# BartvLaatum/GreenLight-Gym2

Hardware: NVIDIA B200
Metric: GreenLight env-steps/sec (fp64 parity) (higher is better)
Workload: dtype f64

## Files before the change

### greenlight-gym2_b200/csrc/glg_kernels.cuh

```cuda
#pragma once
#include <cuda_runtime.h>
#include <stdint.h>

#include "glg_controller.h"
#include "glg_model.h"
#include "glg_philox.h"
#include "glg_rk4.h"

#define GLG_NOBS_FIXED 23
#define GLG_MAXOBSMOD 8
#define GLG_OBS_STATE 1
#define GLG_OBS_CLIMATE 2
#define GLG_OBS_CROP 3
#define GLG_OBS_CONTROL 4
#define GLG_OBS_WEATHER 5
#define GLG_OBS_TIME 6
#define GLG_OBS_FORECAST 7
#define GLG_NOBS_STATE 27
#define GLG_NINFO 11
#define GLG_NSTATS 16

struct GlgUniform {
    double P[GLG_NP];
    double K[K_COUNT];
// ... 160 lines not shown
                if (off + i < 3) o3[off + i] = v;
            }
        } else if (id == GLG_OBS_STATE) {
#pragma unroll 1
            for (int b = 0; b < (GLG_NOBS_STATE + 1) / 2; ++b) {
                const GlgPhilox4 r = glg_philox4x32_10(96u + (uint32_t)b, ctr, (uint32_t)env_id, (uint32_t)(env_id >> 32),
                                                       (uint32_t)A.seed, (uint32_t)(A.seed >> 32));
                const double v0 = glg_u01(r.v[0], r.v[1]), v1 = glg_u01(r.v[2], r.v[3]);
                orow[off + 2 * b] = (float)v0;
                if (hrow) hrow[hoff + 2 * b] = (float)v0;
                if (off + 2 * b < 3) o3[off + 2 * b] = v0;
                if (2 * b + 1 < GLG_NOBS_STATE) {
                    orow[off + 2 * b + 1] = (float)v1;
                    if (hrow) hrow[hoff + 2 * b + 1] = (float)v1;
                    if (off + 2 * b + 1 < 3) o3[off + 2 * b + 1] = v1;
                }
            }
        } else if (id == GLG_OBS_FORECAST) {
#pragma unroll 1
            for (int i = 0; off + i < 3 && i < 5 * A.Np; ++i) o3[off + i] = wnext[(i / 5) * GLG_ND + (i % 5)];
        }
    }
}

__device__ __forceinline__ double glg_warp_sum(double v) {
#pragma unroll
    for (int o = 16; o > 0; o >>= 1) v += __shfl_down_sync(0xffffffffu, v, o);
    return v;
}


__device__ __forceinline__ int glg_stage_weather(const GlgStepArgs &A, double *s_wtile, uint64_t *s_bar, int *s_misc,
                                                 bool active, int kw, int tbl, int &bk, int &bt) {
    if (threadIdx.x == 0) {
        s_misc[0] = kw;
        s_misc[1] = tbl;
        glg_mbar_init(s_bar, 1);
    }
    __syncthreads();
    bk = s_misc[0];
    bt = s_misc[1];
    const int uniform = __syncthreads_and(!active || (kw == bk && tbl == bt));
    if (uniform) {
        const uint32_t tile_bytes = (uint32_t)((A.Np + 1) * GLG_ND * sizeof(double));
        if (threadIdx.x == 0) {
            glg_mbar_expect_tx(s_bar, tile_bytes);
            glg_bulk_g2s(s_wtile, A.weather + ((size_t)bt * A.rows + (size_t)bk) * GLG_ND, tile_bytes, s_bar);
        }
        glg_mbar_wait(s_bar, 0);
    }
    return uniform;
}

template <bool NOISY, class HC, class CC>
__device__ __forceinline__ void glg_env_prologue(const GlgUniform &U, const GlgStepArgs &A, int e, const double *wrow,
                                                 unsigned int ctr, HC &Hc, CC &Cc, double *x, double *u, double *d) {
    const int B = A.B;
#pragma unroll
    for (int i = 0; i < 7; ++i) d[i] = wrow[i];
    if (A.raw_control == 2) {
        double xc[GLG_NX], dc[GLG_ND];
#pragma unroll
        for (int i = 0; i < GLG_NX; ++i) xc[i] = (i == 0 || i == 2 || i == 15) ? A.x[(size_t)i * B + e] : 0.0;
#pragma unroll
        for (int i = 0; i < GLG_ND; ++i) dc[i] = wrow[i];
        glg_rule_control(A.ctrl, xc, dc, A.time[(size_t)B + e], A.time[e], u);
    } else if (A.raw_control) {
#pragma unroll
        for (int i = 0; i < GLG_NU; ++i) u[i] = A.controls[(size_t)e * GLG_NU + i];
    } else {
#pragma unroll
        for (int i = 0; i < GLG_NU; ++i) {
            const float prod = __fmul_rn(A.actions[(size_t)e * GLG_NU + i], A.delta_u_max_f32);
            u[i] = glg_clamp(A.u[(size_t)i * B + e] + (double)prod, A.u_min[i], A.u_max[i]);
        }
    }
#pragma unroll
    for (int i = 0; i < GLG_NU; ++i) A.u[(size_t)i * B + e] = u[i];
#pragma unroll
    for (int i = 0; i < GLG_NX; ++i) x[i] = A.x[(size_t)i * B + e];
    if (NOISY) {
        double pl[GLG_NP];
        double n34[34];
        if (A.noise) {
#pragma unroll 1
            for (int i = 0; i < 34; ++i) n34[i] = A.noise[(size_t)e * 34 + i];
        } else {
            glg_noise34(A.seed, (unsigned long long)(A.env_id_offset + e), ctr, A.uncertainty_scale, n34);
        }
#pragma unroll 1
        for (int i = 0; i < GLG_NP; ++i) pl[i] = U.P[i];
#pragma unroll 1
        for (int i = 0; i < 34; ++i) {
            const double pv = U.P[128 + i];
            pl[128 + i] = (double)__double2float_rn(pv + n34[i] * pv);
        }
        pl[144] = (double)__fdiv_rn(__double2float_rn(pl[141]), __double2float_rn(pl[142]));
        double Cl[C_COUNT];
        glg_make_c(pl, Cl);
#pragma unroll
        for (int i = 0; i < C_COUNT; ++i) Cc[i] = Cl[i];
        glg_hoist(pl, u, d, Hc);
    } else {
        glg_hoist(GlgConstView{U.P}, u, d, Hc);
    }
}

struct GlgEnvOut {
    int done, k_obs, tbl_obs, k_term, tbl_term;
    double fin_ret, fin_len, fin_info[GLG_NINFO];
};

__device__ __forceinline__ void glg_env_epilogue(const GlgUniform &U, const GlgStepArgs &A, int e, int k, int kw, int tbl,
                                                 const double *wrow, double *x, double fruit_prev, int bad,
                                                 unsigned int ctr, GlgEnvOut &o) {
    const int B = A.B;
    const size_t table_stride = (size_t)A.rows * GLG_ND;
    int done = 0;
    if (bad) {
#pragma unroll
        for (int i = 0; i < GLG_NX; ++i) x[i] = A.x[(size_t)i * B + e];
        done = 1;
    }
    double doy = A.time[e], hod = A.time[(size_t)B + e];
    doy += fmod(A.dt / 86400.0, 365.0);
    hod = fmod(hod + A.dt / 3600.0, 24.0);
    double u[GLG_NU], d[GLG_ND];
#pragma unroll
    for (int i = 0; i < GLG_NU; ++i) u[i] = A.u[(size_t)i * B + e];
#pragma unroll
    for (int i = 0; i < 5; ++i) d[i] = wrow[i];
    double hd[GLG_NOBS_FIXED];
    double o3[3] = {0.0, 0.0, 0.0};
    glg_obs_head(x, u, d, k, doy, hod, hd);
    float *orow = A.obs + (size_t)e * A.obs_dim;
    const unsigned long long env_gid = (unsigned long long)(A.env_id_offset + e);
    float *step_row = orow;
    float *hrow = A.obs_head + (size_t)e * (A.obs_dim - (A.fc_off >= 0 ? 5 * A.Np : 0));
    if (k >= A.N) done = 1;
    if (done && A.auto_reset) step_row = A.term_obs + (size_t)e * A.obs_dim;
    glg_write_obs_row(A, hd, wrow + GLG_ND, env_gid, ctr, step_row, step_row == orow ? hrow : nullptr, o3);
    double reward, info[GLG_NINFO];
    {
        const double dt = A.dt;
        const double heat_costs = u[0] * U.P[108] / U.P[46] * dt / 3600 * 1e-3 * A.heating_price;
        const double elec_costs = u[4] * U.P[172] * dt / 3600 * 1e-3 * A.elec_price;
        const double co2_costs = u[1] * U.P[109] / U.P[46] * dt * 1e-6 * A.co2_price;
        const double variable_costs = 0 + heat_costs + co2_costs + elec_costs;
        const double gains = (x[25] - fruit_prev) * 1e-6 / A.dmfm * A.fruit_price;
        const double profit = gains - variable_costs;
        const double max_profit = U.P[154] * dt * 1e-6 / A.dmfm * A.fruit_price;
        const double max_heating = U.P[108] / U.P[46] * dt / 3600 * 1e-3 * A.heating_price;
        const double max_elec = U.P[172] * dt / 3600 * 1e-3 * A.elec_price;
        const double max_co2 = U.P[109] / U.P[46] * dt * 1e-6 * A.co2_price;
        const double min_profit = -(0 + max_heating + max_elec + max_co2);
        const double max_viol[3] = {2500, 15, 15};
        double viol[3], pen = 0.0;
#pragma unroll
// ... 40 lines not shown
        doy = A.start_day[tbl];
        hod = 0.0;
        glg_obs_head(x, u, d, 0, doy, hod, hd);
        double o3r[3];
        glg_write_obs_row(A, hd, w0 + GLG_ND, env_gid, ctr + 0x80000000u, orow, hrow, o3r);
        o.k_obs = 0;
        o.tbl_obs = tbl;
    }
#pragma unroll
    for (int i = 0; i < GLG_NX; ++i) A.x[(size_t)i * B + e] = x[i];
    A.timestep[e] = k;
    A.table[e] = tbl;
    A.time[e] = doy;
    A.time[(size_t)B + e] = hod;
    A.step_ctr[e] = ctr + 1u;
    A.ep_return[e] = done ? 0.0 : ep_ret;
    A.ep_len[e] = done ? 0 : ep_len;
#pragma unroll
    for (int j = 0; j < GLG_NINFO; ++j) A.ep_info[(size_t)j * B + e] = done ? 0.0 : info[j];
    o.done = done;
    o.fin_ret = done ? ep_ret : 0.0;
    o.fin_len = done ? (double)ep_len : 0.0;
#pragma unroll
    for (int j = 0; j < GLG_NINFO; ++j) o.fin_info[j] = done ? info[j] : 0.0;
}

__device__ __forceinline__ void glg_stats_reduce(const GlgStepArgs &A, bool active, int bad, const GlgEnvOut &o) {
    const unsigned any_done = __ballot_sync(0xffffffffu, active && o.done);
    if (!any_done) return;
    const double cnt = glg_warp_sum((active && o.done) ? 1.0 : 0.0);
    const double ret = glg_warp_sum(o.fin_ret);
    const double len = glg_warp_sum(o.fin_len);
    const double nbad = glg_warp_sum((active && bad) ? 1.0 : 0.0);
    double isum[GLG_NINFO];
#pragma unroll
    for (int j = 0; j < GLG_NINFO; ++j) isum[j] = glg_warp_sum(o.fin_info[j]);
    if ((threadIdx.x & 31) == 0) {
        atomicAdd(A.stats + 0, cnt);
        atomicAdd(A.stats + 1, ret);
        atomicAdd(A.stats + 2, len);
#pragma unroll
        for (int j = 0; j < GLG_NINFO; ++j) atomicAdd(A.stats + 3 + j, isum[j]);
        atomicAdd(A.stats + 14, nbad);
    }
}

__device__ __forceinline__ void glg_write_forecast(const GlgStepArgs &A, int NR, const int *s_tbl, const int *s_k,
                                                   const int *s_tbl_t, const int *s_k_t, const double *s_wtile,
                                                   int uniform, int bk, int bt) {
    if (A.fc_off < 0) return;
    const size_t table_stride = (size_t)A.rows * GLG_ND;
    const int nf = 5 * A.Np;
    const int row0 = blockIdx.x * NR;
#pragma unroll 1
    for (int r = 0; r < NR; ++r) {
        const int kk = s_k[r];
        if (kk < 0) continue;
        const int tb = s_tbl[r];
        const double *src = (uniform && tb == bt && kk == bk) ? s_wtile : (A.weather + (size_t)tb * table_stride + (size_t)kk * GLG_ND);
        float *orow = A.obs + (size_t)(row0 + r) * A.obs_dim + A.fc_off;
        for (int j = threadIdx.x; j < nf; j += blockDim.x) {
            const int i = j / 5, c = j - 5 * i;
            orow[j] = (float)src[(size_t)(1 + i) * GLG_ND + c];
        }
        const int kt = s_k_t[r];
        if (kt >= 0) {
            const double *srct = A.weather + (size_t)s_tbl_t[r] * table_stride + (size_t)kt * GLG_ND;
            float *trow = A.term_obs + (size_t)(row0 + r) * A.obs_dim + A.fc_off;
            for (int j = threadIdx.x; j < nf; j += blockDim.x) {
                const int i = j / 5, c = j - 5 * i;
                trow[j] = (float)srct[(size_t)(1 + i) * GLG_ND + c];
            }
        }
    }
}

template <int NT, bool NOISY>
struct GlgStepSmem {
    static constexpr int kColRows = 2 * GLG_NX + H_COUNT + (NOISY ? C_COUNT : 0);
    __host__ __device__ static size_t bytes(int Np) {
        return sizeof(double) * ((size_t)kColRows * NT + (size_t)(Np + 1) * GLG_ND) + 16  + sizeof(int) * (4 * NT + 4);
    }
};

template <bool GENERAL, bool NOISY, int NT>
__global__ void __launch_bounds__(NT) glg_step_kernel(const __grid_constant__ GlgUniform U, const __grid_constant__ GlgStepArgs A) {
    glg_exp_tbl_fill();
    extern __shared__ __align__(16) unsigned char smem_raw[];
    double *s_wtile = reinterpret_cast<double *>(smem_raw);
    double *s_cols = s_wtile + (size_t)(A.Np + 1) * GLG_ND;
    uint64_t *s_bar = reinterpret_cast<uint64_t *>(s_cols + (size_t)GlgStepSmem<NT, NOISY>::kColRows * NT);
    int *s_tbl = reinterpret_cast<int *>(s_bar + 2);
    int *s_k = s_tbl + NT;
    int *s_tbl_t = s_k + NT;
    int *s_k_t = s_tbl_t + NT;
    int *s_misc = s_k_t + NT;

    const int tid = threadIdx.x;
    const int e = blockIdx.x * NT + tid;
    const bool active = e < A.B;
    int k = 0, tbl = 0;
    if (active) {
        k = A.timestep[e];
        tbl = A.table[e];
    }
    const int kw = min(k, A.rows - A.Np - 1);
    int bk, bt;
    const int uniform = glg_stage_weather(A, s_wtile, s_bar, s_misc, active, kw, tbl, bk, bt);

    GlgEnvOut o;
    o.done = 0; o.k_obs = -1; o.tbl_obs = 0; o.k_term = -1; o.tbl_term = 0; o.fin_ret = 0.0; o.fin_len = 0.0;
#pragma unroll
    for (int j = 0; j < GLG_NINFO; ++j) o.fin_info[j] = 0.0;
    int bad = 0;
    if (active) {
        const double *wrow = uniform ? s_wtile : (A.weather + ((size_t)tbl * A.rows + (size_t)kw) * GLG_ND);
        GlgCol<NT> Hc{s_cols + (size_t)(2 * GLG_NX) * NT + tid};
        GlgCol<NT> Cc{s_cols + (size_t)(2 * GLG_NX + H_COUNT) * NT + tid};
        GlgSmemStore<NT> st{s_cols + tid};
        double x[GLG_NX], u[GLG_NU], d[GLG_ND];
        const unsigned int ctr = A.step_ctr[e];
        glg_env_prologue<NOISY>(U, A, e, wrow, ctr, Hc, Cc, x, u, d);
// ... 129 lines not shown
```

### greenlight-gym2_b200/csrc/glg_model.h

```cpp
#pragma once
#include <math.h>

#include <type_traits>
#include <utility>

#include "glg_math.h"

#define GLG_NX 28
#define GLG_NU 6
#define GLG_ND 10
#define GLG_NP 208

enum GlgK {
    K_K1PAR, K_K2PAR, K_KNIR, K_KFIR,
    K_RHOFLRPAR, K_RHOCANNIR, K_RHOFLRNIR, K_TAUHATFLRNIR,
    K_C87, K_C91, K_C92, K_C98, K_C99, K_C100, K_C101,
    K_GHVENT,
    K_RHOC,
    K_HALFG,
    K_RHOCP,
    K_HECIN,
    K_PIPEAIR, K_GROPIPEAIR,
    K_2ALFA,
    K_HFLRSO1, K_HSO12, K_HSO23, K_HSO34, K_HSO45, K_HSO5OUT, K_HCOV, K_HLAMPAIR,
// ... 82 lines not shown
    K[K_HSO34] = fabs(2. * p[103] / (p[29] + p[30]));
    K[K_HSO45] = fabs(2. * p[103] / (p[30] + p[31]));
    K[K_HSO5OUT] = fabs(2. * p[103] / (p[31] + p[37]));
    K[K_HCOV] = fabs(1. / (p[73] / p[71]));
    K[K_HLAMPAIR] = fabs(p[185]);
    K[K_ETAMGPPM] = p[7];
    K[K_VEC] = 2. * p[111] * p[23] / (p[1] * p[14]);
    K[K_RB] = p[41];
    K[K_L] = p[1];
    const double capCov01 = 0.1 * (cos(p[45] * pi / 180.) * p[73] * p[64] * p[72]);
    K[K_INVCAPCO2AIR] = 1. / p[122]; K[K_INVCAPCO2TOP] = 1. / p[123];
    K[K_INVCAPAIR] = 1. / p[112]; K[K_INVCAPTOP] = 1. / p[120];
    K[K_INVCAPLEAF] = 1. / p[16];
    K[K_INVCAPCOV] = 1. / capCov01;
    K[K_INVCAPTHSCR] = 1. / p[119]; K[K_INVCAPFLR] = 1. / p[113]; K[K_INVCAPPIPE] = 1. / p[110];
    K[K_INVCAPSO1] = 1. / p[114]; K[K_INVCAPSO2] = 1. / p[115]; K[K_INVCAPSO3] = 1. / p[116];
    K[K_INVCAPSO4] = 1. / p[117]; K[K_INVCAPSO5] = 1. / p[118];
    K[K_INVVPAIR] = p[39] / (p[38] * p[48]);
    K[K_INVVPTOP] = p[39] / (p[38] * (p[49] - p[48]));
    K[K_INVCAPLAMP] = 1. / p[184]; K[K_INVCAPINTLAMP] = 1. / p[191]; K[K_INVCAPGROPIPE] = 1. / p[171];
    K[K_INVCAPBLSCR] = 1. / p[121];
    K[K_PPMC] = 1e6 * 8.3144598 * 1e-6 / (101325 * 44.01e-3);
    K[K_INVTENDSUM] = 1. / p[163];
}

template <class P>
GLG_HD void glg_make_c(const P &p, double *C) {
    C[C_SLA] = p[142];
    C[C_J25] = p[129];
    C[C_CGAMMA] = p[130];
    C[C_20CGAMMA] = 20 * p[130];
    C[C_ETASTOM] = p[131];
    const double r3 = 1e-3 * p[39];
    C[C_ARR1] = p[132] / (r3 * p[133]);
    C[C_T25K] = p[133];
    C[C_ARR2A] = p[134] / r3;
    C[C_ARR2B] = p[135] / r3;
    C[C_JPOTNUM] = 1 + exp((p[134] * p[133] - p[135]) / (r3 * p[133]));
    C[C_INV2THETA] = 1. / (2. * p[136]);
    C[C_ALPHA] = p[137];
    C[C_4THETAALPHA] = 4 * p[136] * p[137];
    C[C_MCH2O] = p[138];
    C[C_CO2RATIO] = p[139] / p[138];
    C[C_CBUFMAX] = p[157]; C[C_CBUFMIN] = p[158];
    C[C_T24MIN] = p[160]; C[C_T24MAX] = p[159]; C[C_TCANMIN] = p[162]; C[C_TCANMAX] = p[161];
    C[C_RGLEAF] = p[155]; C[C_RGSTEM] = p[156]; C[C_RGFRUIT] = p[154];
    C[C_GLEAF] = p[147]; C[C_GSTEM] = p[148]; C[C_GFRUIT] = p[146];
    C[C_MAINT] = 1. - exp(-p[149] * p[143]);
    C[C_LNQ10X] = 0.1 * log(p[150]);
    C[C_MLEAF] = p[152]; C[C_MSTEM] = p[153]; C[C_MFRUIT] = p[151];
    C[C_CLEAFMAX] = p[144]; C[C_CFRUITMAX] = p[145];
}

template <class P, class HOUT>
GLG_HD void glg_hoist(const P &p, const double *u, const double *d, HOUT &H) {
    const double pi = 3.14159265358979323846;
    const double thScr = u[2], blScr = u[5];
    const double tauThPar = 1 - thScr * (1 - p[80]), rhoThPar = thScr * p[77];
    const double tauA = glg_tau12(p[69], tauThPar, p[66], rhoThPar);
    const double rupA = glg_rhoup(p[69], p[66], p[66], rhoThPar);
    const double rdnA = glg_rhodn(tauThPar, p[66], rhoThPar, rhoThPar);
    const double tauThNir = 1 - thScr * (1 - p[79]), rhoThNir = thScr * p[76];
    const double tauB = glg_tau12(p[68], tauThNir, p[65], rhoThNir);
    const double rupB = glg_rhoup(p[68], p[65], p[65], rhoThNir);
    const double rdnB = glg_rhodn(tauThNir, p[65], rhoThNir, rhoThNir);
    const double tauBlPar = 1 - blScr * (1 - p[90]), rhoBlPar = blScr * p[88];
    const double tauA2 = glg_tau12(tauA, tauBlPar, rdnA, rhoBlPar);
    const double rupA2 = glg_rhoup(tauA, rupA, rdnA, rhoBlPar);
    const double rdnA2 = glg_rhodn(tauBlPar, rdnA, rhoBlPar, rhoBlPar);
    const double tauBlNir = 1 - blScr * (1 - p[89]), rhoBlNir = blScr * p[87];
    const double tauB2 = glg_tau12(tauB, tauBlNir, rdnB, rhoBlNir);
    const double rupB2 = glg_rhoup(tauB, rupB, rdnB, rhoBlNir);
    const double rdnB2 = glg_rhodn(tauBlNir, rdnB, rhoBlNir, rhoBlNir);
    const double tauCovPar = glg_tau12(tauA2, p[176], rdnA2, p[179]);
    const double rhoCovPar = glg_rhoup(tauA2, rupA2, rdnA2, p[179]);
    const double tauCovNir = glg_tau12(tauB2, p[177], rdnB2, p[180]);
    const double rhoCovNir = glg_rhoup(tauB2, rupB2, rdnB2, p[180]);
    const double aCovPar = 1 - tauCovPar - rhoCovPar, aCovNir = 1 - tauCovNir - rhoCovNir;
    const double epsCovFir = 1 - p[70] - p[67];

    const double iGlob = d[0];
    const double qLamp = p[172] * u[4];
    const double parSun = (1 - p[44]) * tauCovPar * p[6] * iGlob;
    const double parLamp = p[174] * qLamp;
    const double rCan = (1 - p[44]) * iGlob * (p[6] * tauCovPar + p[5] * tauCovNir) + (p[174] + p[175]) * qLamp;
    H[H_PARCAN_W] = (parSun + parLamp) * (1 - p[10]);
    H[H_PARLAMP_W] = parLamp * (1 - p[10]);
    H[H_PARFLR_W] = (1 - p[98]) * (parSun + parLamp);
    H[H_PARLAMPFLR_W] = (1 - p[98]) * parLamp;
    H[H_PARUMOL] = (p[187] * parLamp + p[140] * parSun) * (1 - p[10]);
    H[H_RHOCOVNIR] = rhoCovNir;
    H[H_TAUHATCOVNIR] = 1 - rhoCovNir;
    H[H_TAUHAT2] = (1 - rhoCovNir) * (1 - rhoCovNir);
    H[H_NIRSUN] = (1 - p[44]) * p[5] * iGlob;
    H[H_NIRLAMPCAN] = p[175] * qLamp * (1 - p[11]);
    H[H_NIRLAMPFLR] = (1 - p[97]) * p[175] * qLamp;
    H[H_LAMPRAD] = (p[174] + p[175]) * qLamp;
    H[H_GLOBAIR_A] = p[44] * iGlob * tauCovPar * p[6];
    H[H_GLOBAIR_B] = p[44] * iGlob * p[5];
    H[H_GLOBCOV] = (aCovPar * p[6] + aCovNir * p[5]) * iGlob;

    const double sigma = p[2];
    const double tauThFir = 1 - thScr * (1 - p[81]);
    const double tauBlFir = 1 - blScr * (1 - p[91]);
    const double fPipe = 0.49 * pi * p[107] * p[105];
    const double t178 = p[178], t199 = p[199];
    H[H_C84] = p[3] * epsCovFir * (t178 * tauThFir * tauBlFir) * sigma;
    H[H_C86] = p[3] * p[74] * (t178 * thScr * tauBlFir) * sigma;
    H[H_C108] = p[3] * p[85] * (t178 * blScr) * sigma;
    H[H_C88] = p[124] * p[104] * epsCovFir * (t199 * t178 * tauThFir * tauBlFir * 0.49) * sigma;
    H[H_C90] = p[124] * p[104] * p[74] * (t199 * t178 * thScr * tauBlFir * 0.49) * sigma;
    H[H_C93] = p[95] * epsCovFir * (t199 * t178 * tauThFir * tauBlFir * (1 - fPipe)) * sigma;
    H[H_C95] = p[95] * p[74] * (t199 * t178 * thScr * tauBlFir * (1 - fPipe)) * sigma;
    H[H_C106] = p[95] * p[85] * (t199 * t178 * blScr * (1 - fPipe)) * sigma;
    H[H_C107] = p[124] * p[104] * p[85] * (t199 * t178 * blScr * 0.49) * sigma;
    H[H_C96] = p[74] * epsCovFir * thScr * sigma;
    H[H_C102] = p[181] * p[182] * p[74] * (thScr * tauBlFir) * sigma;
    H[H_C103] = p[181] * p[182] * epsCovFir * (tauThFir * tauBlFir) * sigma;
    H[H_C109] = blScr * p[85] * p[74] * thScr * sigma;
    H[H_C110] = blScr * p[85] * epsCovFir * tauThFir * sigma;
    H[H_C112] = p[181] * p[182] * p[85] * blScr * sigma;
    H[H_TSKY4] = glg_sq(glg_sq(d[5] + GLG_C2K));

    const double tOut = d[1], wind = d[4];
    const double aRoofU = u[3] * p[55];
    const double cD = p[59], cW = p[61];
    const double v132a = u[3] * p[55] * cD / (2. * p[46]);
    const double a133 = cD / p[46] * sqrt(1e-8 + (glg_sq(aRoofU) * cW * (wind * wind)));
    const double fLeak = (wind < p[205]) ? p[205] * p[60] : p[60] * wind;
    const double scrMax = fmax(thScr, blScr);
    const bool roofOnly = (1.0 >= p[8]);
    H[H_TOUT] = tOut;
    H[H_TOUT_2K] = tOut + 2 * GLG_C2K;
    H[H_CW_WIND2] = cW * (wind * wind);
    H[H_VR_A] = roofOnly ? p[57] * v132a : p[57] * scrMax * v132a;
    H[H_VR_B] = roofOnly ? p[204] * fLeak : p[57] * (1 - scrMax) * a133 + p[204] * fLeak;
    const double fVentSide = (1 - p[204]) * fLeak;
    H[H_FVENTSIDE_ABS] = fabs(fVentSide);

    H[H_THK] = thScr * p[84];
    H[H_BLK] = blScr * p[94];
    H[H_1MTH] = 1. - thScr;
    H[H_1MBL] = 1. - blScr;

    H[H_17TH] = 1.7 * thScr;
    H[H_17BL] = 1.7 * blScr;
    H[H_HEC_AIROUT] = fabs(p[111] * p[23] * fVentSide);
    H[H_HEC_COVEOUT] = fabs(p[47] / p[46] * (p[51] + p[52] * pow(wind, p[53])));
    H[H_TSOOUT] = d[6];

    const double sRs = 1. / (1. + exp(p[43] * (rCan - p[40])));
    H[H_CEVAP3] = p[20] * (1. - sRs) + p[19] * sRs;
    H[H_CEVAP4] = p[22] * (1. - sRs) + p[21] * sRs;
    H[H_RS] = p[42] * ((rCan + p[17]) / (rCan + p[18]));

    H[H_VPOUT_T] = d[2] / (tOut + (GLG_C2K + GLG_C2K_F32_DELTA));
    H[H_MVAIROUT_C] = 0.002165 * fabs(fVentSide);
    H[H_MCEXT] = u[1] * p[109] / p[46];
    H[H_CO2OUT] = d[3];

    H[H_HBOIL] = u[0] * p[108] / p[46];
    H[H_LAMPNET] = qLamp - (p[174] + p[175]) * qLamp - p[186] * qLamp;
    H[H_HECIN] = p[50] * p[47] / p[46];
    H[H_ZERO] = 0.0;
}

template <bool GENERAL, class KV, class CV, class HV, class P>
GLG_HD double glg_rhs(const KV &K, const CV &C, const HV &H, const P &p, const double *u, const double *d,
                      const double *x, double *S) {
    const double tAir = x[2], tTop = x[3], tCan = x[4], tCovIn = x[5], tCovE = x[6];
    const double tThScr = x[7], tFlr = x[8], tPipe = x[9], tLamp = x[17], tBlScr = x[20];

    {
        const double hFlrSo1 = K[K_HFLRSO1] * (tFlr - x[10]);
        const double hSo12 = K[K_HSO12] * (x[10] - x[11]);
        const double hSo23 = K[K_HSO23] * (x[11] - x[12]);
        const double hSo34 = K[K_HSO34] * (x[12] - x[13]);
        const double hSo45 = K[K_HSO45] * (x[13] - x[14]);
        const double hSo5Out = K[K_HSO5OUT] * (x[14] - H[H_TSOOUT]);
        S[10] = K[K_INVCAPSO1] * (hFlrSo1 - hSo12);
        S[11] = K[K_INVCAPSO2] * (hSo12 - hSo23);
        S[12] = K[K_INVCAPSO3] * (hSo23 - hSo34);
        S[13] = K[K_INVCAPSO4] * (hSo34 - hSo45);
        S[14] = K[K_INVCAPSO5] * (hSo45 - hSo5Out);
        S[21] = (1. / 86400.) * (tCan - x[21]);
        S[26] = (1. / 86400.) * tCan;
        S[27] = 1. / 86400.;
    }
    double sFlr = -(K[K_HFLRSO1] * (tFlr - x[10]));
    double sAir, sTop, sCan, sCovIn, sCovE, sThScr, sPipe, sLamp, sBlScr, sGroPipe, sIntLamp = 0.0;

    const double lai = C[C_SLA] * x[23];
    const double e35 = glg_exp(-K[K_KFIR] * lai);
    const double aCan = 1 - e35;
    double parCan;
    {
        const double e32 = glg_exp(-K[K_K1PAR] * lai);
        const double e33 = GENERAL ? glg_exp(-K[K_K2PAR] * lai) : e32;
        const double e34 = glg_exp(-K[K_KNIR] * lai);
        const double gPar = (1 - e32) + e32 * K[K_RHOFLRPAR] * (1 - e33);
        parCan = H[H_PARUMOL] * gPar;
        const double parLampCanW = H[H_PARLAMP_W] * gPar;
        const double parLampFlrW = H[H_PARLAMPFLR_W] * e32;
        const double rhoCovNir = H[H_RHOCOVNIR];
        const double rhoHat = K[K_RHOCANNIR] * (1 - e34);
        const double den1 = glg_rcp(1. - rhoCovNir * rhoHat);
        const double tCC = H[H_TAUHATCOVNIR] * e34 * den1;
        const double rUp = rhoCovNir + H[H_TAUHAT2] * rhoHat * den1;
        const double rDn = rhoHat + e34 * e34 * rhoCovNir * den1;
        const double den2 = glg_rcp(1. - rDn * K[K_RHOFLRNIR]);
        const double aFlrNir = tCC * K[K_TAUHATFLRNIR] * den2;
        const double rCCF = rUp + tCC * tCC * K[K_RHOFLRNIR] * den2;
        const double aCanNir = 1 - aFlrNir - rCCF;
        const double nirLampCan = H[H_NIRLAMPCAN] * (1 - e34), nirLampFlr = H[H_NIRLAMPFLR] * e34;
        sCan = H[H_PARCAN_W] * gPar + H[H_NIRSUN] * aCanNir + nirLampCan;
        sFlr += H[H_PARFLR_W] * e32 + H[H_NIRSUN] * aFlrNir + nirLampFlr;
        sAir = (H[H_LAMPRAD] - parLampCanW - nirLampCan - parLampFlrW - nirLampFlr)
// ... 270 lines not shown
```

### greenlight-gym2_b200/csrc/glg_roles.cuh

```cuda
#pragma once
#include "glg_kernels.cuh"
#include "glg_units.h"

#define GLG_ROLE_LANES 32
constexpr int GLG_NO = 4;
constexpr int GLG_BAR_PARTS = 1, GLG_BAR_XS = 2, GLG_BAR_LATE = 3;
#ifndef GLG_HREG
#define GLG_HREG 1
#endif
#ifndef GLG_ORDER_TOKEN
#define GLG_ORDER_TOKEN 0
#endif
constexpr int GLG_MAXCONTRIB = 8;
constexpr int GLG_MAXROWS = 8;

#ifdef GLG_TRACE
__device__ long long glg_trace[32][16][2];
#define GLG_TRACE_MARK(warp_, slot_, ev_)                                                          \
    do {                                                                                             \
        if (blockIdx.x == 0 && (threadIdx.x & 31) == 0 && (ev_) >= 64 && (ev_) < 96) glg_trace[(ev_) - 64][warp_][slot_] = clock64(); \
    } while (0)
#else
#define GLG_TRACE_MARK(warp_, slot_, ev_) do {} while (0)
#endif
// ... 443 lines not shown
            });
        }
        if (first) {
            double lam_s = 0.0;
            if (graded) lam_s = glg_stiffness(GlgConstView{U.K}, (double)part_col[PL::ASCR * NL], (double)part_col[PL::AVENT * NL]);
            const bool split = split_h || (graded && (sub < GLG_GRADED_SUBSTEPS || h_nom * lam_s * GLG_STIFF_INV_CFL >= 1.0));
            m_lane = 1;
            m_cta = 1;
            h_lane = h_nom;
            if (__any_sync(0xffffffffu, split)) {
                m_lane = glg_micro_steps_from_lambda((double)part_col[PL::LAMBDA * NL], h_nom);
                if (graded) {
                    int ms = 1 + (int)floor(h_nom * lam_s * GLG_STIFF_INV_CFL);
                    ms = ms > GLG_MAX_MICRO ? GLG_MAX_MICRO : (ms < 1 ? 1 : ms);
                    if (ms < glg_graded_m(sub)) ms = glg_graded_m(sub);
                    m_lane = max(m_lane, ms);
                }
                m_cta = __reduce_max_sync(0xffffffffu, m_lane);
                h_lane = m_lane == 1 ? h_nom : h_nom * glg_rcp((double)m_lane);
                const double hcs = cs * h_lane;
#pragma unroll
                for (int j = 0; j < NJ; ++j) {
                    hc[j] = hcs * scale[j];
                    if (kHasLate) xn[j] = glg_fma(hc[j], sum[j], xo[j]);
                }
            }
            n_micro += m_lane;
        }
        if (!kHasLate) {
#pragma unroll
            for (int j = 0; j < NJ; ++j) xn[j] = glg_fma(hc[j], sum[j], base[j]);
        }
#pragma unroll
        for (int j = 0; j < NJ; ++j) xbase[j * GLG_NO * NL] = (T)xn[j];
    }
    __device__ __forceinline__ int finish(double *s_xfin, int lane) const {
        int bad = 0;
        glg_static_for<0, NJ>([&](auto jc) {
            constexpr int j = decltype(jc)::value;
            const int st = row_state<j>();
            bad |= !(fabs(xn[j]) <= 1.79769313486231570e308);
            if (!kStateInXs && st >= 0) s_xfin[st * NL + lane] = xn[j];
        });
        return bad;
    }
};


template <class T, bool GENERAL, bool NOISY, int NG, int MINB, bool FUSED>
__global__ void __launch_bounds__(32 * (NG + (FUSED ? 0 : GLG_NO)), MINB) glg_step_units_kernel(const __grid_constant__ GlgUniform U,
                                                                                                 const __grid_constant__ GlgStepArgs A) {
    extern __shared__ __align__(16) unsigned char smem_raw[];
    static_assert(!FUSED || NG == GLG_NO, "fused layout: one group role per owner");
    glg_exp_tbl_fill();
    constexpr int NL = GLG_ROLE_LANES;
    constexpr int NT = 32 * (NG + (FUSED ? 0 : GLG_NO));
    using PL = GlgPlan<NG, GENERAL>;
    using SW = GlgSurfaceWarps<NG, GENERAL>;
    constexpr int NJ = PL::NJ;
    double *s_wtile = reinterpret_cast<double *>(smem_raw);
    constexpr int kXfinRows = GlgRoleSmem<T, NG, GENERAL, NOISY>::kXfinRows;
    constexpr bool kStateInXs = kXfinRows == 0;
    double *s_fruit = s_wtile + (size_t)(A.Np + 1) * GLG_ND;
    double *s_scale = s_fruit + NL;
    double *s_xfin = s_scale + NL;
    T *s_xs = reinterpret_cast<T *>(s_xfin + kXfinRows * NL);
    T *s_part = s_xs + PL::XS_ROWS * NL;
    T *s_H = s_part + PL::NSLOTS * NL;
    T *s_C = s_H + H_COUNT * NL;
    uint64_t *s_bar = reinterpret_cast<uint64_t *>(reinterpret_cast<unsigned char *>(s_xs) + GlgRoleSmem<T, NG, GENERAL, NOISY>::col_bytes());
    int *s_tbl = reinterpret_cast<int *>(s_bar + 2);
    int *s_k = s_tbl + NL;
    int *s_tbl_t = s_k + NL;
    int *s_k_t = s_tbl_t + NL;
    int *s_bad = s_k_t + NL;
    int *s_misc = s_bad + NL;
    volatile int *s_stop = s_misc + 4;

    const int tid = threadIdx.x;
    const int lane = tid & 31, warp = tid >> 5;
    const int e = blockIdx.x * A.role_lanes + lane;
    const bool active = lane < A.role_lanes && e < A.B;
    int k = 0, tbl = 0;
    if (active) {
        k = A.timestep[e];
        tbl = A.table[e];
    }
    const int kw = min(k, A.rows - A.Np - 1);
    int bk, bt;
    const int uniform = glg_stage_weather(A, s_wtile, s_bar, s_misc, active, kw, tbl, bk, bt);
    const double *wrow = uniform ? s_wtile : (A.weather + ((size_t)tbl * A.rows + (size_t)kw) * GLG_ND);

    double u[GLG_NU], d[GLG_ND];
#pragma unroll
    for (int i = 0; i < GLG_NU; ++i) u[i] = 0.0;
    double fruit_prev = 0.0;
    unsigned int ctr = 0;
    GlgColT<T, NL> Hc{s_H + lane};
    GlgColT<T, NL> Cc{s_C + lane};
    if (warp == 0) {
        double x[GLG_NX];
        if (active) {
            ctr = A.step_ctr[e];
            glg_env_prologue<NOISY>(U, A, e, wrow, ctr, Hc, Cc, x, u, d);
            fruit_prev = x[25];
        } else {
            double d0[GLG_ND];
#pragma unroll
            for (int i = 0; i < 7; ++i) d0[i] = A.weather[i];
            glg_init_state(d0, x);
            if (NOISY) {
#pragma unroll
                for (int i = 0; i < C_COUNT; ++i) Cc[i] = (T)U.C[i];
            }
            glg_hoist(GlgConstView{U.P}, u, d0, Hc);
        }
        glg_static_for<0, GLG_NX>([&](auto ic) {
            constexpr int i = decltype(ic)::value;
            constexpr int r = PL::plan.rank[i];
            s_xs[r * NL + lane] = (T)x[i];
            if (!kStateInXs) s_xfin[i * NL + lane] = x[i];
        });
        s_fruit[lane] = fruit_prev;
        s_k[lane] = k;
        s_tbl[lane] = tbl;
        s_bad[lane] = 0;
        if (lane < 16) s_stop[lane] = 0;
        if (lane < PL::XS_ROWS) {
            int sk = -1;
            glg_static_for<0, PL::XS_ROWS>([&](auto nc) {
                constexpr int n = decltype(nc)::value;
                constexpr int v = PL::plan.scale_k[n];
                sk = lane == n ? v : sk;
            });
            s_scale[lane] = sk >= 0 ? U.K[sk] : 1.0;
        }
        if (lane == 0) {
            s_misc[2] = uniform;
            s_misc[3] = 0;
        }
    } else {
        for (int i = tid - 32; i < PL::NSLOTS * NL; i += NT - 32) s_part[i] = (T)0;
    }
    __syncthreads();

    T *xs_col = s_xs + lane;
    T *part_col = s_part + lane;
    int n_micro = 0;
    constexpr int kLaunchRegs = (65536 / (MINB * NT)) / 8 * 8 > 255 ? 248 : (65536 / (MINB * NT)) / 8 * 8;
    constexpr int kGroupRegs = kLaunchRegs >= 80 ? 64 : kLaunchRegs >= 64 ? 56 : 48;
    constexpr int kOwnerRegs = (kLaunchRegs + (kLaunchRegs - kGroupRegs) * NG / GLG_NO) / 8 * 8;
    constexpr bool kRebalance = !FUSED && MINB > 1 && kLaunchRegs > kGroupRegs && kLaunchRegs <= 80 && NG % 4 == 0;
    if (FUSED) {
        if (GENERAL && active && warp == GlgWT<NG, GENERAL>::unit_warp(U_FIR)) {
#pragma unroll
            for (int i = 0; i < GLG_NU; ++i) u[i] = A.u[(size_t)i * A.B + e];
        }
        GlgOwner<T, NG, GENERAL> own;
        own.init(warp, A, s_xfin, s_scale, xs_col, lane, false);
#pragma unroll 1
        for (;;) {
            glg_group_eval_dispatch<NG, 0, GENERAL, NOISY, T>(warp, U, xs_col, part_col, s_H + lane, s_C + lane, u);
            own.pre(lane);
            __syncthreads();
            own.post_early(part_col);
            own.post_late(U, part_col, xs_col);
            if (own.final_eval) break;
            own.book();
            __syncthreads();
        }
        n_micro = own.n_micro;
        if (own.finish(s_xfin, lane)) s_bad[lane] = 1;
    } else if (warp >= GLG_NO) {
        if (kRebalance) glg_reg_dec<kGroupRegs>();
        const int gw = warp - GLG_NO;
        if (GENERAL && active && gw == GlgWT<NG, GENERAL>::unit_warp(U_FIR)) {
#pragma unroll
            for (int i = 0; i < GLG_NU; ++i) u[i] = A.u[(size_t)i * A.B + e];
        }
        if (SW::shared && (gw == SW::th || gw == SW::bl || gw == SW::cv)) glg_surface_loop<NG, GENERAL, T>(gw, U, xs_col, part_col, s_H + lane, s_stop, NT);
        else glg_group_dispatch<NG, 0, GENERAL, NOISY, T>(gw, U, xs_col, part_col, s_H + lane, s_C + lane, u, s_stop, NT);
        if (kRebalance) glg_reg_inc<kLaunchRegs>();
    } else {
        if (kRebalance) glg_reg_inc<kOwnerRegs>();
        GlgOwner<T, NG, GENERAL> own;
        own.init(warp, A, s_xfin, s_scale, xs_col, lane, true);
        const int zero = *reinterpret_cast<const volatile int *>(s_misc + 3);
        constexpr int n_early = 32 * (GLG_NO + PL::plan.n_early_warps), n_late = 32 * (GLG_NO + PL::plan.n_late_warps);
        glg_bar_arrive(GLG_BAR_XS, NT);
        [[maybe_unused]] int ev = 0;
#pragma unroll 1
        for (;;) {
            own.book();
            own.pre(lane);
            if (PL::late_mask != 0u) {
// ... 55 lines not shown
```

Before: 5.480 million.

## Spread role-kernel prologue across warps and split hoist into parallel slices

The per-env prologue in the role kernel used to run entirely on warp 0. Now the state load is distributed across all warps, the non-noisy hoist is split into light/FIR/vent slices computed by separate warps, bookkeeping moves to the last warp, and per-env buffers are prefetched into L2 early. The exp table fill is moved after the state loads so that global latency overlaps with it. The forecast writer also assigns one row per warp instead of looping rows with the whole block. The cost is redundant control computation in each hoist warp and more code paths, which may raise register pressure.

```diff
diff --git a/greenlight-gym2_b200/csrc/glg_kernels.cuh b/greenlight-gym2_b200/csrc/glg_kernels.cuh
--- a/greenlight-gym2_b200/csrc/glg_kernels.cuh
+++ b/greenlight-gym2_b200/csrc/glg_kernels.cuh
@@ -236,58 +236,81 @@
     return uniform;
 }
 
+__device__ __forceinline__ void glg_env_control(const GlgStepArgs &A, int e, const double *wrow, double *u) {
+    const int B = A.B;
+    if (A.raw_control == 2) {
+        double xc[GLG_NX], dc[GLG_ND];
+#pragma unroll
+        for (int i = 0; i < GLG_NX; ++i) xc[i] = (i == 0 || i == 2 || i == 15) ? A.x[(size_t)i * B + e] : 0.0;
+#pragma unroll
+        for (int i = 0; i < GLG_ND; ++i) dc[i] = wrow[i];
+        glg_rule_control(A.ctrl, xc, dc, A.time[(size_t)B + e], A.time[e], u);
+    } else if (A.raw_control) {
+#pragma unroll
+        for (int i = 0; i < GLG_NU; ++i) u[i] = A.controls[(size_t)e * GLG_NU + i];
+    } else {
+#pragma unroll
+        for (int i = 0; i < GLG_NU; ++i) {
+            const float prod = __fmul_rn(A.actions[(size_t)e * GLG_NU + i], A.delta_u_max_f32);
+            u[i] = glg_clamp(A.u[(size_t)i * B + e] + (double)prod, A.u_min[i], A.u_max[i]);
+        }
+    }
+}
+
+template <class HC, class CC>
+__device__ __forceinline__ void glg_env_noisy_hoist(const GlgUniform &U, const GlgStepArgs &A, int e, unsigned int ctr, const double *u,
+                                                    const double *d, HC &Hc, CC &Cc) {
+    double pl[GLG_NP];
+    double n34[34];
+    if (A.noise) {
+#pragma unroll 1
+        for (int i = 0; i < 34; ++i) n34[i] = A.noise[(size_t)e * 34 + i];
+    } else {
+        glg_noise34(A.seed, (unsigned long long)(A.env_id_offset + e), ctr, A.uncertainty_scale, n34);
+    }
+#pragma unroll 1
+    for (int i = 0; i < GLG_NP; ++i) pl[i] = U.P[i];
+#pragma unroll 1
+    for (int i = 0; i < 34; ++i) {
+        const double pv = U.P[128 + i];
+        pl[128 + i] = (double)__double2float_rn(pv + n34[i] * pv);
+    }
+    pl[144] = (double)__fdiv_rn(__double2float_rn(pl[141]), __double2float_rn(pl[142]));
+    double Cl[C_COUNT];
+    glg_make_c(pl, Cl);
+#pragma unroll
+    for (int i = 0; i < C_COUNT; ++i) Cc[i] = Cl[i];
+    glg_hoist(pl, u, d, Hc);
+}
+
 template <bool NOISY, class HC, class CC>
 __device__ __forceinline__ void glg_env_prologue(const GlgUniform &U, const GlgStepArgs &A, int e, const double *wrow,
                                                  unsigned int ctr, HC &Hc, CC &Cc, double *x, double *u, double *d) {
     const int B = A.B;
 #pragma unroll
     for (int i = 0; i < 7; ++i) d[i] = wrow[i];
-    if (A.raw_control == 2) {
-        double xc[GLG_NX], dc[GLG_ND];
-#pragma unroll
-        for (int i = 0; i < GLG_NX; ++i) xc[i] = (i == 0 || i == 2 || i == 15) ? A.x[(size_t)i * B + e] : 0.0;
-#pragma unroll
-        for (int i = 0; i < GLG_ND; ++i) dc[i] = wrow[i];
-        glg_rule_control(A.ctrl, xc, dc, A.time[(size_t)B + e], A.time[e], u);
-    } else if (A.raw_control) {
-#pragma unroll
-        for (int i = 0; i < GLG_NU; ++i) u[i] = A.controls[(size_t)e * GLG_NU + i];
-    } else {
-#pragma unroll
-        for (int i = 0; i < GLG_NU; ++i) {
-            const float prod = __fmul_rn(A.actions[(size_t)e * GLG_NU + i], A.delta_u_max_f32);
-            u[i] = glg_clamp(A.u[(size_t)i * B + e] + (double)prod, A.u_min[i], A.u_max[i]);
-        }
-    }
+    glg_env_control(A, e, wrow, u);
 #pragma unroll
     for (int i = 0; i < GLG_NU; ++i) A.u[(size_t)i * B + e] = u[i];
 #pragma unroll
     for (int i = 0; i < GLG_NX; ++i) x[i] = A.x[(size_t)i * B + e];
-    if (NOISY) {
-        double pl[GLG_NP];
-        double n34[34];
-        if (A.noise) {
-#pragma unroll 1
-            for (int i = 0; i < 34; ++i) n34[i] = A.noise[(size_t)e * 34 + i];
-        } else {
-            glg_noise34(A.seed, (unsigned long long)(A.env_id_offset + e), ctr, A.uncertainty_scale, n34);
-        }
-#pragma unroll 1
-        for (int i = 0; i < GLG_NP; ++i) pl[i] = U.P[i];
-#pragma unroll 1
-        for (int i = 0; i < 34; ++i) {
-            const double pv = U.P[128 + i];
-            pl[128 + i] = (double)__double2float_rn(pv + n34[i] * pv);
-        }
-        pl[144] = (double)__fdiv_rn(__double2float_rn(pl[141]), __double2float_rn(pl[142]));
-        double Cl[C_COUNT];
-        glg_make_c(pl, Cl);
-#pragma unroll
-        for (int i = 0; i < C_COUNT; ++i) Cc[i] = Cl[i];
-        glg_hoist(pl, u, d, Hc);
-    } else {
-        glg_hoist(GlgConstView{U.P}, u, d, Hc);
-    }
+    if (NOISY) glg_env_noisy_hoist(U, A, e, ctr, u, d, Hc, Cc);
+    else glg_hoist(GlgConstView{U.P}, u, d, Hc);
+}
+
+__device__ __forceinline__ void glg_prefetch_l2(const void *p) { asm volatile("prefetch.global.L2 [%0];" ::"l"(p)); }
+__device__ __forceinline__ void glg_prefetch_env(const GlgStepArgs &A, int e) {
+    const size_t B = (size_t)A.B;
+    if (A.raw_control == 0) glg_prefetch_l2(A.actions + (size_t)e * GLG_NU);
+#pragma unroll
+    for (int i = 0; i < GLG_NU; ++i) glg_prefetch_l2(A.u + i * B + e);
+    glg_prefetch_l2(A.step_ctr + e);
+    glg_prefetch_l2(A.time + e);
+    glg_prefetch_l2(A.time + B + e);
+    glg_prefetch_l2(A.ep_return + e);
+    glg_prefetch_l2(A.ep_len + e);
+#pragma unroll
+    for (int j = 0; j < GLG_NINFO; ++j) glg_prefetch_l2(A.ep_info + j * B + e);
 }
 
 struct GlgEnvOut {
@@ -434,14 +457,15 @@
     const size_t table_stride = (size_t)A.rows * GLG_ND;
     const int nf = 5 * A.Np;
     const int row0 = blockIdx.x * NR;
-#pragma unroll 1
-    for (int r = 0; r < NR; ++r) {
+    const int lane = threadIdx.x & 31, nwarps = blockDim.x >> 5;
+#pragma unroll 1
+    for (int r = threadIdx.x >> 5; r < NR; r += nwarps) {
         const int kk = s_k[r];
         if (kk < 0) continue;
         const int tb = s_tbl[r];
         const double *src = (uniform && tb == bt && kk == bk) ? s_wtile : (A.weather + (size_t)tb * table_stride + (size_t)kk * GLG_ND);
         float *orow = A.obs + (size_t)(row0 + r) * A.obs_dim + A.fc_off;
-        for (int j = threadIdx.x; j < nf; j += blockDim.x) {
+        for (int j = lane; j < nf; j += 32) {
             const int i = j / 5, c = j - 5 * i;
             orow[j] = (float)src[(size_t)(1 + i) * GLG_ND + c];
         }
@@ -449,7 +473,7 @@
         if (kt >= 0) {
             const double *srct = A.weather + (size_t)s_tbl_t[r] * table_stride + (size_t)kt * GLG_ND;
             float *trow = A.term_obs + (size_t)(row0 + r) * A.obs_dim + A.fc_off;
-            for (int j = threadIdx.x; j < nf; j += blockDim.x) {
+            for (int j = lane; j < nf; j += 32) {
                 const int i = j / 5, c = j - 5 * i;
                 trow[j] = (float)srct[(size_t)(1 + i) * GLG_ND + c];
             }
diff --git a/greenlight-gym2_b200/csrc/glg_model.h b/greenlight-gym2_b200/csrc/glg_model.h
--- a/greenlight-gym2_b200/csrc/glg_model.h
+++ b/greenlight-gym2_b200/csrc/glg_model.h
@@ -158,8 +158,11 @@
     C[C_CLEAFMAX] = p[144]; C[C_CFRUITMAX] = p[145];
 }
 
-template <class P, class HOUT>
-GLG_HD void glg_hoist(const P &p, const double *u, const double *d, HOUT &H) {
+enum GlgHoistSlice { GLG_HOIST_ALL = -1, GLG_HOIST_LIGHT, GLG_HOIST_FIR, GLG_HOIST_VENT, GLG_HOIST_NSLICES };
+template <int S, class P, class HOUT>
+GLG_HD void glg_hoist_slice(const P &p, const double *u, const double *d, HOUT &H) {
+    const bool light = S == GLG_HOIST_ALL || S == GLG_HOIST_LIGHT, fir = S == GLG_HOIST_ALL || S == GLG_HOIST_FIR,
+               vent = S == GLG_HOIST_ALL || S == GLG_HOIST_VENT;
     const double pi = 3.14159265358979323846;
     const double thScr = u[2], blScr = u[5];
     const double tauThPar = 1 - thScr * (1 - p[80]), rhoThPar = thScr * p[77];
@@ -190,43 +193,43 @@
     const double parSun = (1 - p[44]) * tauCovPar * p[6] * iGlob;
     const double parLamp = p[174] * qLamp;
     const double rCan = (1 - p[44]) * iGlob * (p[6] * tauCovPar + p[5] * tauCovNir) + (p[174] + p[175]) * qLamp;
-    H[H_PARCAN_W] = (parSun + parLamp) * (1 - p[10]);
-    H[H_PARLAMP_W] = parLamp * (1 - p[10]);
-    H[H_PARFLR_W] = (1 - p[98]) * (parSun + parLamp);
-    H[H_PARLAMPFLR_W] = (1 - p[98]) * parLamp;
-    H[H_PARUMOL] = (p[187] * parLamp + p[140] * parSun) * (1 - p[10]);
-    H[H_RHOCOVNIR] = rhoCovNir;
-    H[H_TAUHATCOVNIR] = 1 - rhoCovNir;
-    H[H_TAUHAT2] = (1 - rhoCovNir) * (1 - rhoCovNir);
-    H[H_NIRSUN] = (1 - p[44]) * p[5] * iGlob;
-    H[H_NIRLAMPCAN] = p[175] * qLamp * (1 - p[11]);
-    H[H_NIRLAMPFLR] = (1 - p[97]) * p[175] * qLamp;
-    H[H_LAMPRAD] = (p[174] + p[175]) * qLamp;
-    H[H_GLOBAIR_A] = p[44] * iGlob * tauCovPar * p[6];
-    H[H_GLOBAIR_B] = p[44] * iGlob * p[5];
-    H[H_GLOBCOV] = (aCovPar * p[6] + aCovNir * p[5]) * iGlob;
+    if (light) H[H_PARCAN_W] = (parSun + parLamp) * (1 - p[10]);
+    if (light) H[H_PARLAMP_W] = parLamp * (1 - p[10]);
+    if (light) H[H_PARFLR_W] = (1 - p[98]) * (parSun + parLamp);
+    if (light) H[H_PARLAMPFLR_W] = (1 - p[98]) * parLamp;
+    if (light) H[H_PARUMOL] = (p[187] * parLamp + p[140] * parSun) * (1 - p[10]);
+    if (light) H[H_RHOCOVNIR] = rhoCovNir;
+    if (light) H[H_TAUHATCOVNIR] = 1 - rhoCovNir;
+    if (light) H[H_TAUHAT2] = (1 - rhoCovNir) * (1 - rhoCovNir);
+    if (light) H[H_NIRSUN] = (1 - p[44]) * p[5] * iGlob;
+    if (light) H[H_NIRLAMPCAN] = p[175] * qLamp * (1 - p[11]);
+    if (light) H[H_NIRLAMPFLR] = (1 - p[97]) * p[175] * qLamp;
+    if (light) H[H_LAMPRAD] = (p[174] + p[175]) * qLamp;
+    if (light) H[H_GLOBAIR_A] = p[44] * iGlob * tauCovPar * p[6];
+    if (light) H[H_GLOBAIR_B] = p[44] * iGlob * p[5];
+    if (light) H[H_GLOBCOV] = (aCovPar * p[6] + aCovNir * p[5]) * iGlob;
 
     const double sigma = p[2];
     const double tauThFir = 1 - thScr * (1 - p[81]);
     const double tauBlFir = 1 - blScr * (1 - p[91]);
     const double fPipe = 0.49 * pi * p[107] * p[105];
     const double t178 = p[178], t199 = p[199];
-    H[H_C84] = p[3] * epsCovFir * (t178 * tauThFir * tauBlFir) * sigma;
-    H[H_C86] = p[3] * p[74] * (t178 * thScr * tauBlFir) * sigma;
-    H[H_C108] = p[3] * p[85] * (t178 * blScr) * sigma;
-    H[H_C88] = p[124] * p[104] * epsCovFir * (t199 * t178 * tauThFir * tauBlFir * 0.49) * sigma;
-    H[H_C90] = p[124] * p[104] * p[74] * (t199 * t178 * thScr * tauBlFir * 0.49) * sigma;
-    H[H_C93] = p[95] * epsCovFir * (t199 * t178 * tauThFir * tauBlFir * (1 - fPipe)) * sigma;
-    H[H_C95] = p[95] * p[74] * (t199 * t178 * thScr * tauBlFir * (1 - fPipe)) * sigma;
-    H[H_C106] = p[95] * p[85] * (t199 * t178 * blScr * (1 - fPipe)) * sigma;
-    H[H_C107] = p[124] * p[104] * p[85] * (t199 * t178 * blScr * 0.49) * sigma;
-    H[H_C96] = p[74] * epsCovFir * thScr * sigma;
-    H[H_C102] = p[181] * p[182] * p[74] * (thScr * tauBlFir) * sigma;
-    H[H_C103] = p[181] * p[182] * epsCovFir * (tauThFir * tauBlFir) * sigma;
-    H[H_C109] = blScr * p[85] * p[74] * thScr * sigma;
-    H[H_C110] = blScr * p[85] * epsCovFir * tauThFir * sigma;
-    H[H_C112] = p[181] * p[182] * p[85] * blScr * sigma;
-    H[H_TSKY4] = glg_sq(glg_sq(d[5] + GLG_C2K));
+    if (fir) H[H_C84] = p[3] * epsCovFir * (t178 * tauThFir * tauBlFir) * sigma;
+    if (fir) H[H_C86] = p[3] * p[74] * (t178 * thScr * tauBlFir) * sigma;
+    if (fir) H[H_C108] = p[3] * p[85] * (t178 * blScr) * sigma;
+    if (fir) H[H_C88] = p[124] * p[104] * epsCovFir * (t199 * t178 * tauThFir * tauBlFir * 0.49) * sigma;
+    if (fir) H[H_C90] = p[124] * p[104] * p[74] * (t199 * t178 * thScr * tauBlFir * 0.49) * sigma;
+    if (fir) H[H_C93] = p[95] * epsCovFir * (t199 * t178 * tauThFir * tauBlFir * (1 - fPipe)) * sigma;
+    if (fir) H[H_C95] = p[95] * p[74] * (t199 * t178 * thScr * tauBlFir * (1 - fPipe)) * sigma;
+    if (fir) H[H_C106] = p[95] * p[85] * (t199 * t178 * blScr * (1 - fPipe)) * sigma;
+    if (fir) H[H_C107] = p[124] * p[104] * p[85] * (t199 * t178 * blScr * 0.49) * sigma;
+    if (fir) H[H_C96] = p[74] * epsCovFir * thScr * sigma;
+    if (fir) H[H_C102] = p[181] * p[182] * p[74] * (thScr * tauBlFir) * sigma;
+    if (fir) H[H_C103] = p[181] * p[182] * epsCovFir * (tauThFir * tauBlFir) * sigma;
+    if (fir) H[H_C109] = blScr * p[85] * p[74] * thScr * sigma;
+    if (fir) H[H_C110] = blScr * p[85] * epsCovFir * tauThFir * sigma;
+    if (fir) H[H_C112] = p[181] * p[182] * p[85] * blScr * sigma;
+    if (fir) H[H_TSKY4] = glg_sq(glg_sq(d[5] + GLG_C2K));
 
     const double tOut = d[1], wind = d[4];
     const double aRoofU = u[3] * p[55];
@@ -236,39 +239,43 @@
     const double fLeak = (wind < p[205]) ? p[205] * p[60] : p[60] * wind;
     const double scrMax = fmax(thScr, blScr);
     const bool roofOnly = (1.0 >= p[8]);
-    H[H_TOUT] = tOut;
-    H[H_TOUT_2K] = tOut + 2 * GLG_C2K;
-    H[H_CW_WIND2] = cW * (wind * wind);
-    H[H_VR_A] = roofOnly ? p[57] * v132a : p[57] * scrMax * v132a;
-    H[H_VR_B] = roofOnly ? p[204] * fLeak : p[57] * (1 - scrMax) * a133 + p[204] * fLeak;
+    if (vent) H[H_TOUT] = tOut;
+    if (vent) H[H_TOUT_2K] = tOut + 2 * GLG_C2K;
+    if (vent) H[H_CW_WIND2] = cW * (wind * wind);
+    if (vent) H[H_VR_A] = roofOnly ? p[57] * v132a : p[57] * scrMax * v132a;
+    if (vent) H[H_VR_B] = roofOnly ? p[204] * fLeak : p[57] * (1 - scrMax) * a133 + p[204] * fLeak;
     const double fVentSide = (1 - p[204]) * fLeak;
-    H[H_FVENTSIDE_ABS] = fabs(fVentSide);
-
-    H[H_THK] = thScr * p[84];
-    H[H_BLK] = blScr * p[94];
-    H[H_1MTH] = 1. - thScr;
-    H[H_1MBL] = 1. - blScr;
-
-    H[H_17TH] = 1.7 * thScr;
-    H[H_17BL] = 1.7 * blScr;
-    H[H_HEC_AIROUT] = fabs(p[111] * p[23] * fVentSide);
-    H[H_HEC_COVEOUT] = fabs(p[47] / p[46] * (p[51] + p[52] * pow(wind, p[53])));
-    H[H_TSOOUT] = d[6];
+    if (vent) H[H_FVENTSIDE_ABS] = fabs(fVentSide);
+
+    if (fir) H[H_THK] = thScr * p[84];
+    if (fir) H[H_BLK] = blScr * p[94];
+    if (fir) H[H_1MTH] = 1. - thScr;
+    if (fir) H[H_1MBL] = 1. - blScr;
+
+    if (fir) H[H_17TH] = 1.7 * thScr;
+    if (fir) H[H_17BL] = 1.7 * blScr;
+    if (vent) H[H_HEC_AIROUT] = fabs(p[111] * p[23] * fVentSide);
+    if (vent) H[H_HEC_COVEOUT] = fabs(p[47] / p[46] * (p[51] + p[52] * pow(wind, p[53])));
+    if (fir) H[H_TSOOUT] = d[6];
 
     const double sRs = 1. / (1. + exp(p[43] * (rCan - p[40])));
-    H[H_CEVAP3] = p[20] * (1. - sRs) + p[19] * sRs;
-    H[H_CEVAP4] = p[22] * (1. - sRs) + p[21] * sRs;
-    H[H_RS] = p[42] * ((rCan + p[17]) / (rCan + p[18]));
-
-    H[H_VPOUT_T] = d[2] / (tOut + (GLG_C2K + GLG_C2K_F32_DELTA));
-    H[H_MVAIROUT_C] = 0.002165 * fabs(fVentSide);
-    H[H_MCEXT] = u[1] * p[109] / p[46];
-    H[H_CO2OUT] = d[3];
-
-    H[H_HBOIL] = u[0] * p[108] / p[46];
-    H[H_LAMPNET] = qLamp - (p[174] + p[175]) * qLamp - p[186] * qLamp;
-    H[H_HECIN] = p[50] * p[47] / p[46];
-    H[H_ZERO] = 0.0;
+    if (light) H[H_CEVAP3] = p[20] * (1. - sRs) + p[19] * sRs;
+    if (light) H[H_CEVAP4] = p[22] * (1. - sRs) + p[21] * sRs;
+    if (light) H[H_RS] = p[42] * ((rCan + p[17]) / (rCan + p[18]));
+
+    if (vent) H[H_VPOUT_T] = d[2] / (tOut + (GLG_C2K + GLG_C2K_F32_DELTA));
+    if (vent) H[H_MVAIROUT_C] = 0.002165 * fabs(fVentSide);
+    if (fir) H[H_MCEXT] = u[1] * p[109] / p[46];
+    if (fir) H[H_CO2OUT] = d[3];
+
+    if (fir) H[H_HBOIL] = u[0] * p[108] / p[46];
+    if (light) H[H_LAMPNET] = qLamp - (p[174] + p[175]) * qLamp - p[186] * qLamp;
+    if (fir) H[H_HECIN] = p[50] * p[47] / p[46];
+    if (fir) H[H_ZERO] = 0.0;
+}
+template <class P, class HOUT>
+GLG_HD void glg_hoist(const P &p, const double *u, const double *d, HOUT &H) {
+    glg_hoist_slice<GLG_HOIST_ALL>(p, u, d, H);
 }
 
 template <bool GENERAL, class KV, class CV, class HV, class P>
diff --git a/greenlight-gym2_b200/csrc/glg_roles.cuh b/greenlight-gym2_b200/csrc/glg_roles.cuh
--- a/greenlight-gym2_b200/csrc/glg_roles.cuh
+++ b/greenlight-gym2_b200/csrc/glg_roles.cuh
@@ -519,7 +519,6 @@
                                                                                                  const __grid_constant__ GlgStepArgs A) {
     extern __shared__ __align__(16) unsigned char smem_raw[];
     static_assert(!FUSED || NG == GLG_NO, "fused layout: one group role per owner");
-    glg_exp_tbl_fill();
     constexpr int NL = GLG_ROLE_LANES;
     constexpr int NT = 32 * (NG + (FUSED ? 0 : GLG_NO));
     using PL = GlgPlan<NG, GENERAL>;
@@ -548,47 +547,81 @@
     const int lane = tid & 31, warp = tid >> 5;
     const int e = blockIdx.x * A.role_lanes + lane;
     const bool active = lane < A.role_lanes && e < A.B;
+    constexpr int NW = NT / 32;
+    constexpr int kXRows = (GLG_NX + NW - 1) / NW;
     int k = 0, tbl = 0;
     if (active) {
         k = A.timestep[e];
         tbl = A.table[e];
     }
+    double xw[kXRows];
+    glg_static_for<0, GLG_NX>([&](auto ic) {
+        constexpr int i = decltype(ic)::value;
+        if (warp == i % NW) xw[i / NW] = active ? A.x[(size_t)i * A.B + e] : 0.0;
+    });
+    if (active && warp == NW - 1) glg_prefetch_env(A, e);
+    glg_exp_tbl_fill();
     const int kw = min(k, A.rows - A.Np - 1);
     int bk, bt;
     const int uniform = glg_stage_weather(A, s_wtile, s_bar, s_misc, active, kw, tbl, bk, bt);
     const double *wrow = uniform ? s_wtile : (A.weather + ((size_t)tbl * A.rows + (size_t)kw) * GLG_ND);
 
-    double u[GLG_NU], d[GLG_ND];
-#pragma unroll
-    for (int i = 0; i < GLG_NU; ++i) u[i] = 0.0;
-    double fruit_prev = 0.0;
-    unsigned int ctr = 0;
-    GlgColT<T, NL> Hc{s_H + lane};
-    GlgColT<T, NL> Cc{s_C + lane};
-    if (warp == 0) {
-        double x[GLG_NX];
-        if (active) {
-            ctr = A.step_ctr[e];
-            glg_env_prologue<NOISY>(U, A, e, wrow, ctr, Hc, Cc, x, u, d);
-            fruit_prev = x[25];
-        } else {
-            double d0[GLG_ND];
-#pragma unroll
-            for (int i = 0; i < 7; ++i) d0[i] = A.weather[i];
-            glg_init_state(d0, x);
-            if (NOISY) {
-#pragma unroll
-                for (int i = 0; i < C_COUNT; ++i) Cc[i] = (T)U.C[i];
-            }
-            glg_hoist(GlgConstView{U.P}, u, d0, Hc);
-        }
+    double d0[GLG_ND];
+#pragma unroll
+    for (int i = 0; i < 7; ++i) d0[i] = active ? 0.0 : A.weather[i];
+    {
+        double x0[GLG_NX];
+        if (!active) glg_init_state(d0, x0);
         glg_static_for<0, GLG_NX>([&](auto ic) {
             constexpr int i = decltype(ic)::value;
             constexpr int r = PL::plan.rank[i];
-            s_xs[r * NL + lane] = (T)x[i];
-            if (!kStateInXs) s_xfin[i * NL + lane] = x[i];
+            if (warp == i % NW) {
+                const double v = active ? xw[i / NW] : x0[i];
+                s_xs[r * NL + lane] = (T)v;
+                if (!kStateInXs) s_xfin[i * NL + lane] = v;
+                if (i == 25) s_fruit[lane] = active ? v : 0.0;
+            }
         });
-        s_fruit[lane] = fruit_prev;
+    }
+    for (int i = tid; i < PL::NSLOTS * NL; i += NT) s_part[i] = (T)0;
+    double u[GLG_NU];
+#pragma unroll
+    for (int i = 0; i < GLG_NU; ++i) u[i] = 0.0;
+    GlgColT<T, NL> Hc{s_H + lane};
+    GlgColT<T, NL> Cc{s_C + lane};
+    constexpr bool kSplitHoist = !NOISY && !FUSED;
+    static_assert(!kSplitHoist || NW > GLG_HOIST_NSLICES, "one warp per hoisting slice and one for the bookkeeping");
+    if (kSplitHoist ? warp < GLG_HOIST_NSLICES : warp == 0) {
+        double uc[GLG_NU], d[GLG_ND];
+#pragma unroll
+        for (int i = 0; i < GLG_NU; ++i) uc[i] = 0.0;
+#pragma unroll
+        for (int i = 0; i < 7; ++i) d[i] = active ? wrow[i] : d0[i];
+        if (active) {
+            glg_env_control(A, e, wrow, uc);
+            if (warp == 0) {
+#pragma unroll
+                for (int i = 0; i < GLG_NU; ++i) A.u[(size_t)i * A.B + e] = uc[i];
+            }
+        }
+        if (NOISY) {
+            if (active) {
+                glg_env_noisy_hoist(U, A, e, A.step_ctr[e], uc, d, Hc, Cc);
+            } else {
+#pragma unroll
+                for (int i = 0; i < C_COUNT; ++i) Cc[i] = (T)U.C[i];
+                glg_hoist(GlgConstView{U.P}, uc, d, Hc);
+            }
+        } else if (!kSplitHoist) {
+            glg_hoist(GlgConstView{U.P}, uc, d, Hc);
+        } else if (warp == GLG_HOIST_LIGHT) {
+            glg_hoist_slice<GLG_HOIST_LIGHT>(GlgConstView{U.P}, uc, d, Hc);
+        } else if (warp == GLG_HOIST_FIR) {
+            glg_hoist_slice<GLG_HOIST_FIR>(GlgConstView{U.P}, uc, d, Hc);
+        } else {
+            glg_hoist_slice<GLG_HOIST_VENT>(GlgConstView{U.P}, uc, d, Hc);
+        }
+    } else if (warp == NW - 1) {
         s_k[lane] = k;
         s_tbl[lane] = tbl;
         s_bad[lane] = 0;
@@ -606,8 +639,6 @@
             s_misc[2] = uniform;
             s_misc[3] = 0;
         }
-    } else {
-        for (int i = tid - 32; i < PL::NSLOTS * NL; i += NT - 32) s_part[i] = (T)0;
     }
     __syncthreads();
 
```

Result: faster. 5.586 million (median of 6 runs) (+1.9%).
